# play-with-HOI-generation/HOIG

Hardware: AMD Instinct MI355X
Metric: HOGAN train images/sec at 256x256 (higher is better)
Workload: dtype f16x3 fwd (both operands split hi+lo on fp16, 3 MFMAs per product) / bf16x2 bwd (dy split hi+lo, weights and x single bf16, 2 MFMAs per product), f32 accumulate; 1 GPU; 256x256 HO3Dv3-shaped synthetic, batch 8 per GPU, G+D full step (generator_spade_attn, VGG19 surrogate weights); global_batch=8, parallelism=dp1

## Files before the change

hoig_amd/csrc/conv_thin.hip:

```cpp
#include "common.h"
#include <map>
#include <mutex>

namespace {

typedef _Float16 f16x8 __attribute__((ext_vector_type(8)));
typedef short s16x4 __attribute__((ext_vector_type(4)));

constexpr int TH = 4, TW = 32, NTHR = 256;

struct ThinArgs {
    const float *T;
    const float *D;
    const float *bias;
    float *Out;
    float *Ws;
    int Bn, H, W, F, CD, KS, pad;
    int flip;
    int sj, st, sf;
    int act;
    float slope;
    int accumulate;
    float wscale;
    int K, KP, N, NP;
    int tiles_x, tiles_y, ntiles, strip;
    int HR, CW;
    double *stats;
};

template <bool FP16>
__device__ __forceinline__ void split16(float x, unsigned short &hi, unsigned short &lo) {
    if (FP16) {
        const _Float16 h = (_Float16)x;
        const _Float16 l = (_Float16)(x - (float)h);
        hi = __builtin_bit_cast(unsigned short, h);
        lo = __builtin_bit_cast(unsigned short, l);
    } else {
        const __bf16 h = (__bf16)x;
        hi = __builtin_bit_cast(unsigned short, h);
        const __bf16 l = (__bf16)(x - hoig_bf2f(hi));
        lo = __builtin_bit_cast(unsigned short, l);
    }
}

template <bool FP16>
__device__ __forceinline__ f32x16 mfma16(const bf16x8 a, const bf16x8 b, const f32x16 c) {
    if (FP16) return __builtin_amdgcn_mfma_f32_32x32x16_f16(__builtin_bit_cast(f16x8, a), __builtin_bit_cast(f16x8, b), c, 0, 0, 0);
    return __builtin_amdgcn_mfma_f32_32x32x16_bf16(a, b, c, 0, 0, 0);
}

constexpr int HMAX = 12;
struct HaloRegs {
    float v[HMAX];
};
struct HaloMap {
    int lds[HMAX];
    int rc[HMAX];
    int rounds;
};
__device__ __forceinline__ void halo_map(const ThinArgs &p, HaloMap &m) {
    const int wr = TW + p.KS - 1;
    const int row_elems = wr * p.F;
    const int total = p.HR * row_elems;
    m.rounds = (total + NTHR - 1) / NTHR;
#pragma unroll
    for (int it = 0; it < HMAX; ++it) {
        const int i = threadIdx.x + it * NTHR;
        m.lds[it] = -1;
        m.rc[it] = 0;
        if (i < total) {
            const int hy = i / row_elems, e = i - hy * row_elems;
            const int hx = e / p.F, f = e - hx * p.F;
            m.lds[it] = (f * p.HR + hy) * p.CW + hx;
            m.rc[it] = hy | (hx << 8) | (f << 16);
        }
    }
}
__device__ __forceinline__ void halo_load(const ThinArgs &p, const HaloMap &m, int b, int y0, int x0, HaloRegs &h) {
    const float *img = p.T + (size_t)b * p.H * p.W * p.F;
#pragma unroll
    for (int it = 0; it < HMAX; ++it) {
        h.v[it] = 0.f;
        if (it < m.rounds && m.lds[it] >= 0) {
// ... 83 lines not shown
    const int t_end = min(p.ntiles, (int)(blockIdx.x + 1) * p.strip);
    HaloRegs hreg;
    HaloMap hmap;
    halo_map(p, hmap);
    {
        int b, y0, x0;
        tile_coords(p, blockIdx.x * p.strip, b, y0, x0);
        halo_load(p, hmap, b, y0, x0, hreg);
    }
    float st1[2] = {0.f, 0.f}, st2[2] = {0.f, 0.f};
    int sb = -1;
    auto flush_stats = [&]() {
        if (sb >= 0) {
#pragma unroll
            for (int j = 0; j < 2; ++j) {
                const float s1 = st1[j] + __shfl_xor(st1[j], 32), s2 = st2[j] + __shfl_xor(st2[j], 32);
                if (lh == 0) {
                    hoig_stats_add(p.stats, sb, p.CD, 0, cbase + j * 32 + l31, s1);
                    hoig_stats_add(p.stats, sb, p.CD, 1, cbase + j * 32 + l31, s2);
                }
                st1[j] = st2[j] = 0.f;
            }
        }
    };
    for (int t = blockIdx.x * p.strip; t < t_end; ++t) {
        int b, y0, x0;
        tile_coords(p, t, b, y0, x0);
        if (p.stats && b != sb) {
            flush_stats();
            sb = b;
        }
        __syncthreads();
        halo_store<FP16, NT>(p, hmap, hreg, Tl);
        __syncthreads();
        if (t + 1 < t_end) {
            int b2, y2, x2;
            tile_coords(p, t + 1, b2, y2, x2);
            halo_load(p, hmap, b2, y2, x2, hreg);
        }
        f32x16 acc[2];
#pragma unroll
        for (int j = 0; j < 2; ++j)
#pragma unroll
            for (int r = 0; r < 16; ++r) acc[j][r] = 0.f;
#pragma unroll 1
        for (int kk = 0; kk < ksteps; ++kk) {
            const int k0 = kk * 16 + lh * 8;
            const bf16x8 offs = *reinterpret_cast<const bf16x8 *>(toff + k0);
            bf16x8 a0, a1;
#pragma unroll
            for (int e = 0; e < 8; ++e) {
                const int o = (int)(unsigned short)offs[e] + pix;
                a0[e] = (short)Tl[o];
                if (NT == 2) a1[e] = (short)Tl[tplane + o];
            }
#pragma unroll
            for (int j = 0; j < 2; ++j) {
                const unsigned short *wr = Wl + (j * 32 + l31) * wstride + k0;
                const bf16x8 w0 = *reinterpret_cast<const bf16x8 *>(wr);
                if (NT == 2) acc[j] = mfma16<FP16>(a1, w0, acc[j]);
                if (NW == 2) acc[j] = mfma16<FP16>(a0, *reinterpret_cast<const bf16x8 *>(wr + 64 * wstride), acc[j]);
                acc[j] = mfma16<FP16>(a0, w0, acc[j]);
            }
        }
        const int oy = y0 + wave;
#pragma unroll
        for (int r = 0; r < 16; ++r) {
            const int ox = x0 + (r & 3) + 8 * (r >> 2) + 4 * lh;
            float *dst = p.Out + (((size_t)b * p.H + oy) * p.W + ox) * p.CD + cbase + l31;
#pragma unroll
            for (int j = 0; j < 2; ++j) {
                float v = acc[j][r] * inv + bias_r[j];
                v = fast_act(v, nslope, special, p.act, p.slope);
                if (p.accumulate) v += dst[j * 32];
                dst[j * 32] = v;
                st1[j] += v;
                st2[j] += v * v;
            }
        }
    }
    if (p.stats) flush_stats();
}

constexpr int DROW = 192;

template <int NPW, int WN, int NT, int ND>
__global__ __launch_bounds__(NTHR) void thin_wgrad_kernel(const ThinArgs p) {
    constexpr int WK = 4 / WN, NPIX = TH * TW, KSTEPS = NPIX / 16;
    extern __shared__ __attribute__((aligned(16))) unsigned char smem[];
    unsigned char *Dl = smem;
    unsigned short *Tl = reinterpret_cast<unsigned short *>(smem + ND * NPIX * DROW);
    float *Gl = reinterpret_cast<float *>(smem);
    const int tid = threadIdx.x, lane = tid & 63, wave = tid >> 6;
    const int l31 = lane & 31, lh = lane >> 5;
    const int wn = wave % WN, wk = wave / WN;
    const int cbase = blockIdx.y * 64;
    const int KK = p.KS * p.KS;
    const int tplane = p.F * p.HR * p.CW;

    int noff[NPW];
    bool nval[NPW];
#pragma unroll
    for (int j = 0; j < NPW; ++j) {
        const int n = (wn * NPW + j) * 32 + l31;
        nval[j] = n < p.N;
        const int nc = nval[j] ? n : 0;
        const int tap = nc / p.F, f = nc - tap * p.F;
        const int tt = p.flip ? KK - 1 - tap : tap;
        const int r = tt / p.KS, s = tt - r * p.KS;
        noff[j] = (f * p.HR + r) * p.CW + s + lh * 8;
    }
    const int g = lane >> 4, q = (lane >> 2) & 3, pp = lane & 3;
    const int a_off = (8 * (g >> 1) + q) * DROW + (16 * (g & 1) + 4 * pp) * 2;

    f32x16 acc[2][NPW];
#pragma unroll
    for (int i = 0; i < 2; ++i)
#pragma unroll
        for (int j = 0; j < NPW; ++j)
#pragma unroll
            for (int r = 0; r < 16; ++r) acc[i][j][r] = 0.f;

    constexpr int DT = NPIX * 8 / NTHR;
    float4 dreg[DT][2];
    auto load_d = [&](int t) {
        int b, y0, x0;
        tile_coords(p, t, b, y0, x0);
#pragma unroll
        for (int i = 0; i < DT; ++i) {
            const int task = tid + i * NTHR, px = task >> 3, c8 = task & 7;
            const int yy = y0 + (px >> 5), xx = x0 + (px & 31);
            const float *src = p.D + (((size_t)b * p.H + yy) * p.W + xx) * p.CD + cbase + c8 * 8;
            dreg[i][0] = *reinterpret_cast<const float4 *>(src);
            dreg[i][1] = *reinterpret_cast<const float4 *>(src + 4);
        }
    };
    auto store_d = [&]() {
#pragma unroll
        for (int i = 0; i < DT; ++i) {
            const int task = tid + i * NTHR, px = task >> 3, c8 = task & 7;
            const float v[8] = {dreg[i][0].x, dreg[i][0].y, dreg[i][0].z, dreg[i][0].w,
                                dreg[i][1].x, dreg[i][1].y, dreg[i][1].z, dreg[i][1].w};
            bf16x8 hi, lo;
#pragma unroll
            for (int e = 0; e < 8; e += 2) {
                typedef float f2v __attribute__((ext_vector_type(2)));
                typedef __bf16 b2v __attribute__((ext_vector_type(2)));
                const f2v x2 = {v[e], v[e + 1]};
                const unsigned hp = __builtin_bit_cast(unsigned, __builtin_convertvector(x2, b2v));
                hi[e] = (short)(hp & 0xffffu);
                hi[e + 1] = (short)(hp >> 16);
                if (ND == 2) {
                    const f2v r2 = {v[e] - __uint_as_float(hp << 16), v[e + 1] - __uint_as_float(hp & 0xffff0000u)};
                    const unsigned lp = __builtin_bit_cast(unsigned, __builtin_convertvector(r2, b2v));
                    lo[e] = (short)(lp & 0xffffu);
                    lo[e + 1] = (short)(lp >> 16);
                }
            }
            *reinterpret_cast<bf16x8 *>(Dl + px * DROW + c8 * 16) = hi;
            if (ND == 2) *reinterpret_cast<bf16x8 *>(Dl + NPIX * DROW + px * DROW + c8 * 16) = lo;
        }
    };

    int t = blockIdx.x;
    HaloRegs hreg;
    HaloMap hmap;
// ... 27 lines not shown
                    const s16x4 v0 = __builtin_amdgcn_ds_read_tr16_b64_v4i16((__attribute__((address_space(3))) s16x4 *)(src));
                    const s16x4 v1 = __builtin_amdgcn_ds_read_tr16_b64_v4i16((__attribute__((address_space(3))) s16x4 *)(src + 4 * DROW));
                    a[i][d] = (bf16x8){v0[0], v0[1], v0[2], v0[3], v1[0], v1[1], v1[2], v1[3]};
                }
            const int base = prow * p.CW + pcol;
#pragma unroll
            for (int j = 0; j < NPW; ++j) {
                bf16x8 b0, b1;
#pragma unroll
                for (int e = 0; e < 8; ++e) {
                    const int o = base + noff[j] + e;
                    b0[e] = nval[j] ? (short)Tl[o] : (short)0;
                    if (NT == 2) b1[e] = nval[j] ? (short)Tl[tplane + o] : (short)0;
                }
#pragma unroll
                for (int i = 0; i < 2; ++i) {
                    if (ND == 2) acc[i][j] = mfma16<false>(a[i][1], b0, acc[i][j]);
                    if (NT == 2) acc[i][j] = mfma16<false>(a[i][0], b1, acc[i][j]);
                    acc[i][j] = mfma16<false>(a[i][0], b0, acc[i][j]);
                }
            }
        }
    }

    __syncthreads();
    for (int i = tid; i < 64 * p.NP; i += NTHR) Gl[i] = 0.f;
    __syncthreads();
#pragma unroll
    for (int i = 0; i < 2; ++i)
#pragma unroll
        for (int j = 0; j < NPW; ++j) {
            const int n = (wn * NPW + j) * 32 + l31;
            if (n < p.NP)
#pragma unroll
                for (int r = 0; r < 16; ++r) {
                    const int m = i * 32 + (r & 3) + 8 * (r >> 2) + 4 * lh;
                    if (WK > 1) atomicAdd(&Gl[m * p.NP + n], acc[i][j][r]);
                    else Gl[m * p.NP + n] = acc[i][j][r];
                }
        }
    __syncthreads();
    if (p.Ws) {
        float *dst = p.Ws + ((size_t)blockIdx.y * gridDim.x + blockIdx.x) * 64 * p.NP;
        for (int i = tid; i < 64 * p.NP; i += NTHR) dst[i] = Gl[i];
        return;
    }
    if (p.sj == 1) {
        for (int i = tid; i < 64 * p.N; i += NTHR) {
            const int n = i >> 6, m = i & 63;
            const int tap = n / p.F, f = n - tap * p.F;
            atomicAdd(p.Out + (size_t)f * p.sf + (size_t)tap * p.st + cbase + m, Gl[m * p.NP + n]);
        }
    } else {
        for (int i = tid; i < 64 * p.N; i += NTHR) {
            const int m = i / p.N, n = i - m * p.N;
            const int tap = n / p.F, f = n - tap * p.F;
            atomicAdd(p.Out + (size_t)(cbase + m) * p.sj + (size_t)tap * p.st + (size_t)f * p.sf, Gl[m * p.NP + n]);
        }
    }
}

__global__ __launch_bounds__(NTHR) void thin_reduce_kernel(const ThinArgs p, int nwg) {
    const int cbase = blockIdx.y * 64;
    const float *src = p.Ws + (size_t)blockIdx.y * nwg * 64 * p.NP;
    const int i = blockIdx.x * NTHR + threadIdx.x;
    if (i >= 64 * p.N) return;
    const int m = i / p.N, n = i - m * p.N;
    const int wper = (nwg + (int)gridDim.z - 1) / (int)gridDim.z;
    const int w0 = blockIdx.z * wper, w1 = min(nwg, w0 + wper);
    const size_t step = (size_t)64 * p.NP;
    const float *col = src + m * p.NP + n + (size_t)w0 * step;
    float v0 = 0.f, v1 = 0.f, v2 = 0.f, v3 = 0.f;
    int w = w0;
    for (; w + 3 < w1; w += 4, col += 4 * step) {
        v0 += col[0];
        v1 += col[step];
        v2 += col[2 * step];
        v3 += col[3 * step];
    }
    for (; w < w1; ++w, col += step) v0 += col[0];
    const float v = (v0 + v1) + (v2 + v3);
    const int tap = n / p.F, f = n - tap * p.F;
    atomicAdd(p.Out + (size_t)(cbase + m) * p.sj + (size_t)tap * p.st + (size_t)f * p.sf, v);
}

constexpr size_t WS_SLOT_BYTES = (size_t)16 << 20;
float *thin_workspace(hipStream_t st, size_t bytes) { return static_cast<float *>(hoig_detail::stream_scratch(st, bytes)); }

typedef float f32x4v __attribute__((ext_vector_type(4)));

struct ThinOutArgs {
    const float *D, *Wt, *bias;
    float *Out;
    int Bn, H, W, F, CD, KS, pad, flip;
    int sf, st, sj;
    unsigned long long acts;
    float slope, wscale;
    int tiles_x, tiles_y, ntiles, strip, HR, HWc;
};

template <bool FP16>
__device__ __forceinline__ f32x4v mfma16x16(const bf16x8 a, const bf16x8 b, const f32x4v c) {
    if (FP16) return __builtin_amdgcn_mfma_f32_16x16x32_f16(__builtin_bit_cast(f16x8, a), __builtin_bit_cast(f16x8, b), c, 0, 0, 0);
    return __builtin_amdgcn_mfma_f32_16x16x32_bf16(a, b, c, 0, 0, 0);
}

template <bool FP16, int ND, int NW>
__global__ __launch_bounds__(NTHR) void thin_out_kernel(const ThinOutArgs p) {
    constexpr int PROW = 80, WROW = 144;
    extern __shared__ __attribute__((aligned(16))) unsigned char smem[];
    const int KK = p.KS * p.KS, hpix = p.HR * p.HWc;
    unsigned char *Wl = smem;
    unsigned char *Dl = smem + (size_t)NW * (p.CD >> 6) * p.F * KK * WROW;
    const int tid = threadIdx.x, lane = tid & 63, wave = tid >> 6;
    const int l15 = lane & 15, kg = lane >> 4;
    const int wplane = p.F * KK * WROW;

    for (int i0 = tid; i0 < p.F * KK * p.CD; i0 += 4 * NTHR) {
        float v[4];
        int dst[4];
#pragma unroll
        for (int u = 0; u < 4; ++u) {
            const int i = i0 + u * NTHR;
            v[u] = 0.f;
            dst[u] = -1;
            if (i < p.F * KK * p.CD) {
                const int j = i % p.CD, ft = i / p.CD;
                const int tap = ft % KK, f = ft / KK;
                const int tw = p.flip ? KK - 1 - tap : tap;
                v[u] = p.Wt[(size_t)f * p.sf + (size_t)tw * p.st + (size_t)j * p.sj];
                dst[u] = ((j >> 6) * p.F * KK + f * KK + tap) * WROW + (j & 63) * 2;
            }
        }
#pragma unroll
        for (int u = 0; u < 4; ++u)
            if (dst[u] >= 0) {
                unsigned short hi, lo;
                split16<FP16>(v[u] * p.wscale, hi, lo);
                *reinterpret_cast<unsigned short *>(Wl + dst[u]) = hi;
                if (NW == 2) *reinterpret_cast<unsigned short *>(Wl + (size_t)(p.CD >> 6) * wplane + dst[u]) = lo;
            }
    }

    int apix[2];
#pragma unroll
    for (int i = 0; i < 2; ++i) {
        const int g = 2 * wave + i;
        apix[i] = ((g >> 1) * p.HWc + 16 * (g & 1) + l15) * PROW + kg * 16;
    }
    const bool nvalid = l15 < p.F;
    const int wrow0 = l15 * KK * WROW + kg * 16;
    const float inv = 1.f / p.wscale;
    const int act_n = (int)((p.acts >> (4 * l15)) & 15);
    const float bias_n = (p.bias && nvalid) ? p.bias[l15] : 0.f;

    constexpr int HT = 12;
    float4 hreg[HT];
    auto halo_load = [&](int t, int kh) {
        int b, y0, x0;
        const int tx = t % p.tiles_x, r1 = t / p.tiles_x;
        b = r1 / p.tiles_y;
        y0 = (r1 % p.tiles_y) * TH;
        x0 = tx * TW;
#pragma unroll
        for (int it = 0; it < HT; ++it) {
            const int i = tid + it * NTHR;
// ... 39 lines not shown
            if (kh + 1 < nkh) halo_load(t, kh + 1);
            else if (t + 1 < t_end) halo_load(t + 1, 0);
            const unsigned char *wbase = Wl + (size_t)(kh >> 1) * wplane + wrow0 + (kh & 1) * 64;
#pragma unroll 1
            for (int tap = 0; tap < KK; ++tap) {
                const int r = tap / p.KS, s_ = tap - r * p.KS;
                const int toff = (r * p.HWc + s_) * PROW;
                bf16x8 bh = {0, 0, 0, 0, 0, 0, 0, 0}, bl = bh;
                if (nvalid) {
                    bh = *reinterpret_cast<const bf16x8 *>(wbase + tap * WROW);
                    if (NW == 2) bl = *reinterpret_cast<const bf16x8 *>(wbase + (size_t)(p.CD >> 6) * wplane + tap * WROW);
                }
#pragma unroll
                for (int i = 0; i < 2; ++i) {
                    const unsigned char *ap = Dl + apix[i] + toff;
                    const bf16x8 ah = *reinterpret_cast<const bf16x8 *>(ap);
                    if (ND == 2) acc[i] = mfma16x16<FP16>(*reinterpret_cast<const bf16x8 *>(ap + hpix * PROW), bh, acc[i]);
                    if (NW == 2) acc[i] = mfma16x16<FP16>(ah, bl, acc[i]);
                    acc[i] = mfma16x16<FP16>(ah, bh, acc[i]);
                }
            }
        }
        if (nvalid) {
            const int tx = t % p.tiles_x, r1 = t / p.tiles_x;
            const int b = r1 / p.tiles_y, y0 = (r1 % p.tiles_y) * TH, x0 = tx * TW;
#pragma unroll
            for (int i = 0; i < 2; ++i) {
                const int g = 2 * wave + i;
                const int oy = y0 + (g >> 1), oxb = x0 + 16 * (g & 1) + 4 * kg;
#pragma unroll
                for (int e = 0; e < 4; ++e) {
                    const float v = acc[i][e] * inv + bias_n;
                    p.Out[(((size_t)b * p.H + oy) * p.W + oxb + e) * p.F + l15] = hoig_act(v, act_n, p.slope);
                }
            }
        }
    }
}

bool thin_geometry(const hoig_conv_desc *d) {
    return !d->transposed && d->stride == 1 && d->R == d->S && (d->R & 1) && d->R <= 7 && 2 * d->pad == d->R - 1 &&
           d->Ho == d->Hi && d->Wo == d->Wi && (d->Hi % TH) == 0 && (d->Wi % TW) == 0;
}

void fill_common(ThinArgs &a, const hoig_conv_desc *d, int F, int CD) {
    a.Bn = d->B; a.H = d->Hi; a.W = d->Wi; a.F = F; a.CD = CD; a.KS = d->R; a.pad = d->pad;
    a.K = d->R * d->S * F;
    a.KP = (a.K + 15) / 16 * 16;
    a.N = a.K;
    a.NP = (a.N + 31) / 32 * 32;
    a.tiles_x = d->Wi / TW; a.tiles_y = d->Hi / TH;
    a.ntiles = d->B * a.tiles_x * a.tiles_y;
    a.HR = TH + d->R - 1;
    a.CW = (TW + d->R - 1 + 8 + 1) & ~1;
    a.bias = nullptr; a.act = HOIG_ACT_NONE; a.slope = 0.f; a.accumulate = 0; a.wscale = 1.f; a.strip = 1; a.Ws = nullptr; a.stats = nullptr;
}

template <bool FP16>
int launch_gemm(const ThinArgs &a, int precision, hipStream_t st) {
    const int nt = precision == HOIG_PREC_BF16 ? 1 : 2, nw = precision == HOIG_PREC_BF16X3 ? 2 : 1;
    const size_t smem = (size_t)nw * 64 * (a.KP + 8) * 2 + (size_t)a.KP * 2 + (size_t)nt * a.F * a.HR * a.CW * 2;
    if (smem > 160 * 1024) return HOIG_EUNSUPPORTED;
    dim3 grid((unsigned)hoig_cdiv(a.ntiles, a.strip), a.CD / 64);
    HOIG_ROUTE_FD(FP16, thin);
#define HOIG_THIN_GEMM(NT_, NW_)                                                                                         \
    do {                                                                                                                 \
        static hoig_once attr;                                                                                        \
        if (!attr.done()) {                                                                                                     \
            if (hipFuncSetAttribute(reinterpret_cast<const void *>(&thin_gemm_kernel<FP16, NT_, NW_>),                   \
                                    hipFuncAttributeMaxDynamicSharedMemorySize, 160 * 1024) != hipSuccess)               \
                return HOIG_ELAUNCH;                                                                                     \
            attr.set();                                                                                                 \
        }                                                                                                                \
        thin_gemm_kernel<FP16, NT_, NW_><<<grid, NTHR, smem, st>>>(a);                                                   \
    } while (0)
    if (nt == 2 && nw == 2) HOIG_THIN_GEMM(2, 2);
    else if (nt == 2) HOIG_THIN_GEMM(2, 1);
    else HOIG_THIN_GEMM(1, 1);
#undef HOIG_THIN_GEMM
    HOIG_LAUNCH_CHECK();
    return HOIG_OK;
}

template <int NPW, int WN>
int launch_wgrad_t(const ThinArgs &a, int nt, int nd, dim3 grid, size_t smem, hipStream_t st) {
#define HOIG_THIN_WG(NT_, ND_)                                                                                           \
    do {                                                                                                                 \
        static hoig_once attr;                                                                                        \
        if (!attr.done()) {                                                                                                     \
            if (hipFuncSetAttribute(reinterpret_cast<const void *>(&thin_wgrad_kernel<NPW, WN, NT_, ND_>),               \
                                    hipFuncAttributeMaxDynamicSharedMemorySize, 160 * 1024) != hipSuccess)               \
                return HOIG_ELAUNCH;                                                                                     \
            attr.set();                                                                                                 \
        }                                                                                                                \
        thin_wgrad_kernel<NPW, WN, NT_, ND_><<<grid, NTHR, smem, st>>>(a);                                               \
    } while (0)
    if (nt == 2 && nd == 2) HOIG_THIN_WG(2, 2);
    else if (nt == 2) HOIG_THIN_WG(2, 1);
    else if (nd == 2) HOIG_THIN_WG(1, 2);
    else HOIG_THIN_WG(1, 1);
#undef HOIG_THIN_WG
    HOIG_LAUNCH_CHECK();
    return HOIG_OK;
}

}

int hoig_conv_thin_fwd(const hoig_conv_desc *d, const float *x, const float *w, const float *bias, float *y, hipStream_t st, double *stats) {
    if (d->precision == HOIG_PREC_F32 || !thin_geometry(d) || d->Ci > (d->R <= 3 ? 12 : 8) || d->Ci < 1 || (d->Co % 64)) return HOIG_EUNSUPPORTED;
    ThinArgs a;
    fill_common(a, d, d->Ci, d->Co);
    a.T = x; a.D = w; a.bias = bias; a.Out = y; a.stats = stats;
    a.flip = 0;
    a.sj = d->R * d->S * d->Ci; a.st = d->Ci; a.sf = 1;
    a.act = d->act; a.slope = d->slope;
    a.wscale = 256.f;
    a.strip = a.ntiles >= 4096 ? 8 : (a.ntiles >= 1024 ? 4 : 1);
    return launch_gemm<true>(a, d->precision, st);
}

int hoig_conv_thin_dgrad(const hoig_conv_desc *d, const float *dy, const float *w, float *dx, int accumulate, hipStream_t st) {
    if (d->precision == HOIG_PREC_F32 || !thin_geometry(d) || d->Co > 8 || d->Co < 1 || (d->Ci % 64)) return HOIG_EUNSUPPORTED;
    ThinArgs a;
    fill_common(a, d, d->Co, d->Ci);
    a.T = dy; a.D = w; a.Out = dx;
    a.flip = 1;
    a.sj = 1; a.st = d->Ci; a.sf = d->R * d->S * d->Ci;
    a.accumulate = accumulate;
    a.strip = a.ntiles >= 4096 ? 8 : (a.ntiles >= 1024 ? 4 : 1);
    return launch_gemm<false>(a, d->precision, st);
}

bool hoig_conv_thin_wgrad_applies(const hoig_conv_desc *d) {
    if (d->precision == HOIG_PREC_F32 || !thin_geometry(d)) return false;
    return (d->Ci <= (d->R <= 3 ? 12 : 8) && (d->Co % 64) == 0) || (d->Co <= 8 && (d->Ci % 64) == 0);
}

int hoig_conv_thin_wgrad(const hoig_conv_desc *d, const float *x, const float *dy, float *dw, hipStream_t st) {
    if (d->precision == HOIG_PREC_F32 || !thin_geometry(d)) return HOIG_EUNSUPPORTED;
    const bool thin_in = d->Ci <= (d->R <= 3 ? 12 : 8) && (d->Co % 64) == 0, thin_out = d->Co <= 8 && (d->Ci % 64) == 0;
    if (!thin_in && !thin_out) return HOIG_EUNSUPPORTED;
    ThinArgs a;
    int nt, nd;
    if (thin_in) {
        fill_common(a, d, d->Ci, d->Co);
        a.T = x; a.D = dy; a.flip = 0;
        a.sj = d->R * d->S * d->Ci; a.st = d->Ci; a.sf = 1;
        nd = d->precision == HOIG_PREC_BF16 ? 1 : 2;
        nt = d->precision == HOIG_PREC_BF16X3 ? 2 : 1;
    } else {
        fill_common(a, d, d->Co, d->Ci);
        a.T = dy; a.D = x; a.flip = 1;
        a.sj = 1; a.st = d->Ci; a.sf = d->R * d->S * d->Ci;
        nt = d->precision == HOIG_PREC_BF16 ? 1 : 2;
        nd = d->precision == HOIG_PREC_BF16X3 ? 2 : 1;
    }
    a.Out = dw;
    const int nfr = a.NP / 32;
    if (nfr > 16) return HOIG_EUNSUPPORTED;
    size_t smem = (size_t)nd * TH * TW * DROW + (size_t)nt * a.F * a.HR * a.CW * 2;
    const size_t gsm = (size_t)64 * a.NP * 4;
    if (gsm > smem) smem = gsm;
    if (smem > 160 * 1024) return HOIG_EUNSUPPORTED;
    int nwg = 512;
    if (smem > 80 * 1024 || a.N >= 128) nwg = 256;
    if (nwg > a.ntiles) nwg = a.ntiles;
    const int groups = a.CD / 64;
    while (nwg > 64 && (size_t)nwg * groups * 64 * a.NP * 4 > WS_SLOT_BYTES) nwg >>= 1;
    dim3 grid(nwg, groups);
    a.Ws = nwg > 8 ? thin_workspace(st, (size_t)nwg * groups * 64 * a.NP * 4) : nullptr;
    if (thin_in) a.Ws ? HOIG_ROUTE_W(wgrad_thin_in_ws) : HOIG_ROUTE_W(wgrad_thin_in_direct);
    else a.Ws ? HOIG_ROUTE_W(wgrad_thin_out_ws) : HOIG_ROUTE_W(wgrad_thin_out_direct);
    int rc;
    if (nfr == 1) rc = launch_wgrad_t<1, 1>(a, nt, nd, grid, smem, st);
    else if (nfr == 2) rc = launch_wgrad_t<2, 1>(a, nt, nd, grid, smem, st);
    else if (nfr <= 4) rc = launch_wgrad_t<2, 2>(a, nt, nd, grid, smem, st);
    else if (nfr <= 8) rc = launch_wgrad_t<2, 4>(a, nt, nd, grid, smem, st);
    else rc = launch_wgrad_t<4, 4>(a, nt, nd, grid, smem, st);
    if (rc != HOIG_OK || !a.Ws) return rc;
    thin_reduce_kernel<<<dim3((unsigned)hoig_cdiv(64 * a.N, NTHR), groups, (unsigned)hoig_cdiv(nwg, 32)), NTHR, 0, st>>>(a, nwg);
    HOIG_LAUNCH_CHECK();
    return HOIG_OK;
}

int hoig_conv_thin_out(const hoig_conv_desc *d, const float *x, const float *w, const float *bias, float *y,
                       unsigned long long acts, int dgrad, hipStream_t st) {
    if (d->precision == HOIG_PREC_F32 || !thin_geometry(d)) return HOIG_EUNSUPPORTED;
    const int F = dgrad ? d->Ci : d->Co, CD = dgrad ? d->Co : d->Ci;
    if (F < 1 || F > 16 || (CD % 64)) return HOIG_EUNSUPPORTED;
    if (d->R > 3) return HOIG_EUNSUPPORTED;
    ThinOutArgs a;
    a.D = x; a.Wt = w; a.bias = bias; a.Out = y;
    a.Bn = d->B; a.H = d->Hi; a.W = d->Wi; a.F = F; a.CD = CD; a.KS = d->R; a.pad = d->pad;
    const int KK = d->R * d->S;
    if (!dgrad) { a.flip = 0; a.sf = KK * CD; a.st = CD; a.sj = 1; a.wscale = 256.f; }
    else { a.flip = 1; a.sf = 1; a.st = F; a.sj = KK * F; a.wscale = 1.f; }
    a.acts = acts; a.slope = d->slope;
    a.tiles_x = d->Wi / TW; a.tiles_y = d->Hi / TH; a.ntiles = d->B * a.tiles_x * a.tiles_y;
    a.strip = a.ntiles >= 2048 ? 8 : (a.ntiles >= 512 ? 2 : 1);
    a.HR = TH + d->R - 1; a.HWc = TW + d->R - 1;
    if (a.HR * a.HWc * 8 > 12 * NTHR) return HOIG_EUNSUPPORTED;
    const int nd = d->precision == HOIG_PREC_BF16 ? 1 : 2, nw = d->precision == HOIG_PREC_BF16X3 ? 2 : 1;
    const size_t smem = (size_t)nw * (CD / 64) * F * KK * 144 + (size_t)nd * a.HR * a.HWc * 80;
    if (smem > 160 * 1024) return HOIG_EUNSUPPORTED;
    const unsigned grid = (unsigned)hoig_cdiv(a.ntiles, a.strip);
    HOIG_ROUTE_FD(!dgrad, thin_out);
#define HOIG_THIN_OUT(FP16_, ND_, NW_)                                                                                   \
    do {                                                                                                                 \
        static hoig_once attr;                                                                                        \
        if (!attr.done()) {                                                                                                     \
            if (hipFuncSetAttribute(reinterpret_cast<const void *>(&thin_out_kernel<FP16_, ND_, NW_>),                   \
                                    hipFuncAttributeMaxDynamicSharedMemorySize, 160 * 1024) != hipSuccess)               \
                return HOIG_ELAUNCH;                                                                                     \
            attr.set();                                                                                                 \
        }                                                                                                                \
        thin_out_kernel<FP16_, ND_, NW_><<<grid, NTHR, smem, st>>>(a);                                                   \
    } while (0)
    if (!dgrad) {
        if (nd == 2 && nw == 2) HOIG_THIN_OUT(true, 2, 2);
        else if (nd == 2) HOIG_THIN_OUT(true, 2, 1);
        else HOIG_THIN_OUT(true, 1, 1);
    } else {
        if (nd == 2 && nw == 2) HOIG_THIN_OUT(false, 2, 2);
        else if (nd == 2) HOIG_THIN_OUT(false, 2, 1);
        else HOIG_THIN_OUT(false, 1, 1);
    }
#undef HOIG_THIN_OUT
    HOIG_LAUNCH_CHECK();
    return HOIG_OK;
}
```

hoig_amd/csrc/tuning.h:

```cpp
#pragma once
enum HoigTuning { HOIG_TUNE_IGEMM16 = 0, HOIG_TUNE_S2_16, HOIG_TUNE_FLAT5, HOIG_TUNE_WFLAT5, HOIG_TUNE_HEAD16, HOIG_TUNE_D_EARLY, HOIG_TUNE_SPLIT_GRADS, HOIG_TUNE_PAIR, HOIG_TUNE_WDMA16, HOIG_TUNE_S2_PIPE, HOIG_TUNE_NORM_IN, HOIG_TUNE_WINO8, HOIG_TUNE_HALO5, HOIG_TUNE_COUNT };
int hoig_tuning(int id);
```

hoig_amd/csrc/tuning.hip:

```cpp
#include <cstring>
#include "hoig_kernels.h"
#include "tuning.h"
#include "conv_route.h"

namespace {
struct Entry {
    const char *key;
    int value;
};
Entry g_table[HOIG_TUNE_COUNT] = {
    {"igemm16", 1},
    {"s2_16", 1},
    {"flat5", 2},
    {"wflat5", 1},
    {"head16", 1},
    {"d_early", 1},
    {"split_grads", 1},
    {"pair", 2},
    {"wdma16", 2},
    {"s2_pipe", 1},
    {"norm_in", 1},
    {"wino8", 0},
    {"halo5", 1},
};
}

int hoig_tuning(int id) { return (id >= 0 && id < HOIG_TUNE_COUNT) ? g_table[id].value : 0; }

extern "C" int hoig_set_tuning(const char *key, int value) {
    if (!key) return -1;
    for (int i = 0; i < HOIG_TUNE_COUNT; ++i)
        if (strcmp(g_table[i].key, key) == 0) {
            const int prev = g_table[i].value;
            if (value >= 0) g_table[i].value = value;
            return prev;
        }
    return -1;
}

thread_local int hoig_route_last[3] = {0, 0, 0};

extern "C" int hoig_conv_last_route(int which) { return (which >= 0 && which < 3) ? hoig_route_last[which] : -1; }

extern "C" const char *hoig_conv_route_name(int id) {
    static const char *const names[HOIG_ROUTE_COUNT] = {
        "none",
#define HOIG_R_W(n) #n,
#define HOIG_R_D(n) "dgrad_" #n,
#define HOIG_R_F(n) "fwd_" #n,
#define HOIG_R_FD(n) "fwd_" #n, "dgrad_" #n,
        HOIG_CONV_ROUTES(HOIG_R_W, HOIG_R_D, HOIG_R_F, HOIG_R_FD)
#undef HOIG_R_W
#undef HOIG_R_D
#undef HOIG_R_F
#undef HOIG_R_FD
    };
    return (id >= 0 && id < HOIG_ROUTE_COUNT) ? names[id] : nullptr;
}
```

Measured before the change: 131.1 images/s.

## Add thin16 padded-channel layout kernels for thin conv fwd, dgrad and wgrad

Adds a new family of thin-channel convolution kernels that pad the small channel count to 4/8/16 and pack the halo into a row-contiguous LDS layout. Forward and dgrad use 16x16x32 MFMAs with 512 threads, 8-row tiles and register-prefetched halos, while wgrad uses transposed LDS reads over the new layout. The goal is fewer wasted K-steps and cheaper fragment loads for low-channel convs. The cost is extra padding work, more LDS, and a selection table (thin16_selected) that gates which shapes take the new path.

```diff
diff --git a/hoig_amd/csrc/conv_thin.hip b/hoig_amd/csrc/conv_thin.hip
--- a/hoig_amd/csrc/conv_thin.hip
+++ b/hoig_amd/csrc/conv_thin.hip
@@ -1,4 +1,6 @@
 #include "common.h"
+#include "conv_thin16_tables.h"
+#include "tuning.h"
 #include <map>
 #include <mutex>
 
@@ -248,6 +250,244 @@
     if (p.stats) flush_stats();
 }
 
+constexpr int TH16 = 8, NTHR16 = 512;
+
+typedef unsigned int u32x2 __attribute__((ext_vector_type(2)));
+
+template <bool A16>
+__device__ __forceinline__ bf16x8 lds_frag(const unsigned short *src) {
+    if (A16) return *reinterpret_cast<const bf16x8 *>(src);
+    const u32x2 v0 = *reinterpret_cast<const u32x2 *>(src), v1 = *reinterpret_cast<const u32x2 *>(src + 4);
+    typedef unsigned int u32x4 __attribute__((ext_vector_type(4)));
+    return __builtin_bit_cast(bf16x8, (u32x4){v0[0], v0[1], v1[0], v1[1]});
+}
+
+template <bool FP16>
+__device__ __forceinline__ f32x4 mfma16x32(const bf16x8 a, const bf16x8 b, const f32x4 c) {
+    if (FP16) return __builtin_amdgcn_mfma_f32_16x16x32_f16(__builtin_bit_cast(f16x8, a), __builtin_bit_cast(f16x8, b), c, 0, 0, 0);
+    return __builtin_amdgcn_mfma_f32_16x16x32_bf16(a, b, c, 0, 0, 0);
+}
+
+constexpr int HMAX16 = 9;
+template <int HM>
+struct Halo16 {
+    float v[HM];
+    int rc[HM];
+};
+template <int NTH, int HM>
+__device__ __forceinline__ void halo16_map(const ThinArgs &p, const Thin16Geom &g, Halo16<HM> &m) {
+    const int wr = TW + p.KS - 1;
+    const int row_elems = wr * p.F;
+    const int total = g.HR * row_elems;
+#pragma unroll
+    for (int it = 0; it < HM; ++it) {
+        const int i = threadIdx.x + it * NTH;
+        m.rc[it] = -1;
+        if (i < total) {
+            const int hy = i / row_elems, e = i - hy * row_elems;
+            const int hx = e / p.F, f = e - hx * p.F;
+            m.rc[it] = hy | (hx << 8) | (f << 16);
+        }
+    }
+}
+template <int HM>
+__device__ __forceinline__ void halo16_load(const ThinArgs &p, Halo16<HM> &m, int b, int y0, int x0) {
+    const float *img = p.T + (size_t)b * p.H * p.W * p.F;
+#pragma unroll
+    for (int it = 0; it < HM; ++it) {
+        m.v[it] = 0.f;
+        if (m.rc[it] >= 0) {
+            const int gy = y0 - p.pad + (m.rc[it] & 255), gx = x0 - p.pad + ((m.rc[it] >> 8) & 255);
+            if (gy >= 0 && gy < p.H && gx >= 0 && gx < p.W) m.v[it] = img[((size_t)gy * p.W + gx) * p.F + (m.rc[it] >> 16)];
+        }
+    }
+}
+template <bool FP16, int NT, int HM>
+__device__ __forceinline__ void halo16_store(const Thin16Geom &g, const Halo16<HM> &m, unsigned short *Tl, int plane) {
+#pragma unroll
+    for (int it = 0; it < HM; ++it)
+        if (m.rc[it] >= 0) {
+            unsigned short hi, lo;
+            split16<FP16>(m.v[it], hi, lo);
+            const int o = thin16_halo_elem(g, m.rc[it] & 255, (m.rc[it] >> 8) & 255, m.rc[it] >> 16);
+            Tl[o] = hi;
+            if (NT == 2) Tl[plane + o] = lo;
+        }
+}
+
+template <bool FP16, int NT, int NW, bool A16, bool STATS>
+__global__ __launch_bounds__(NTHR16) void thin16_gemm_kernel(const ThinArgs p, const Thin16Geom g) {
+    extern __shared__ __attribute__((aligned(16))) unsigned char smem[];
+    const int wstride = g.KP + 8;
+    unsigned short *Wl = reinterpret_cast<unsigned short *>(smem);
+    unsigned short *Tl = Wl + NW * 64 * wstride;
+    const int tid = threadIdx.x, lane = tid & 63, wave = tid >> 6;
+    const int l15 = lane & 15, lg = lane >> 4;
+    const int cbase = blockIdx.y * 64;
+    const int tplane = g.HR * g.CWE;
+
+    for (int i0 = tid; i0 < 64 * g.KP; i0 += 4 * NTHR16) {
+        float v[4];
+        int dst[4];
+#pragma unroll
+        for (int u = 0; u < 4; ++u) {
+            const int i = i0 + u * NTHR16;
+            v[u] = 0.f;
+            dst[u] = -1;
+            if (i < 64 * g.KP) {
+                const int n = i / g.KP, k = i - n * g.KP;
+                dst[u] = n * wstride + k;
+                const long long src = thin16_weight_index(g, k, cbase + n, p.sj, p.st, p.sf, p.flip);
+                if (src >= 0) v[u] = p.D[src];
+            }
+        }
+#pragma unroll
+        for (int u = 0; u < 4; ++u)
+            if (dst[u] >= 0) {
+                unsigned short hi, lo;
+                split16<FP16>(v[u] * p.wscale, hi, lo);
+                Wl[dst[u]] = hi;
+                if (NW == 2) Wl[64 * wstride + dst[u]] = lo;
+            }
+    }
+    for (int i = tid; i < NT * tplane; i += NTHR16) Tl[i] = 0;
+
+    const float nslope = p.act == HOIG_ACT_NONE ? 1.f : (p.act == HOIG_ACT_RELU ? 0.f : p.slope);
+    const bool special = p.act == HOIG_ACT_TANH || p.act == HOIG_ACT_SIGMOID;
+    const float inv = 1.f / p.wscale;
+    const int ksteps = g.KP >> 5, spr = g.KRP >> 5;
+    const unsigned short *wlane = Wl + l15 * wstride + lg * 8;
+    const unsigned short *tlane = Tl + wave * g.CWE + l15 * g.FP + lg * 8;
+
+    const int t_end = min(p.ntiles, (int)(blockIdx.x + 1) * p.strip);
+    Halo16<HMAX16> halo;
+    halo16_map<NTHR16>(p, g, halo);
+    auto coords = [&](int t, int &b, int &y0, int &x0) {
+        const int tx = t % p.tiles_x;
+        t /= p.tiles_x;
+        b = t / p.tiles_y;
+        y0 = (t - b * p.tiles_y) * TH16;
+        x0 = tx * TW;
+    };
+    {
+        int b, y0, x0;
+        coords(blockIdx.x * p.strip, b, y0, x0);
+        halo16_load(p, halo, b, y0, x0);
+    }
+    float st1[4][4], st2[4][4];
+#pragma unroll
+    for (int mt = 0; mt < 4; ++mt)
+#pragma unroll
+        for (int e = 0; e < 4; ++e) st1[mt][e] = st2[mt][e] = 0.f;
+    int sb = -1;
+    auto flush_stats = [&]() {
+        if (STATS && sb >= 0) {
+#pragma unroll
+            for (int mt = 0; mt < 4; ++mt)
+#pragma unroll
+                for (int e = 0; e < 4; ++e) {
+                    float s1 = st1[mt][e], s2 = st2[mt][e];
+#pragma unroll
+                    for (int o = 1; o < 16; o <<= 1) {
+                        s1 += __shfl_xor(s1, o);
+                        s2 += __shfl_xor(s2, o);
+                    }
+                    if (l15 == 0) {
+                        hoig_stats_add(p.stats, sb, p.CD, 0, cbase + mt * 16 + lg * 4 + e, s1);
+                        hoig_stats_add(p.stats, sb, p.CD, 1, cbase + mt * 16 + lg * 4 + e, s2);
+                    }
+                    st1[mt][e] = st2[mt][e] = 0.f;
+                }
+        }
+    };
+    struct Frags {
+        bf16x8 w[4][NW], t[2][NT];
+    };
+    for (int t = blockIdx.x * p.strip; t < t_end; ++t) {
+        int b, y0, x0;
+        coords(t, b, y0, x0);
+        if (STATS && b != sb) {
+            flush_stats();
+            sb = b;
+        }
+        __syncthreads();
+        halo16_store<FP16, NT>(g, halo, Tl, tplane);
+        __syncthreads();
+        if (t + 1 < t_end) {
+            int b2, y2, x2;
+            coords(t + 1, b2, y2, x2);
+            halo16_load(p, halo, b2, y2, x2);
+        }
+        const int oy = y0 + wave;
+        if (oy >= p.H) continue;
+        f32x4 acc[4][2];
+#pragma unroll
+        for (int mt = 0; mt < 4; ++mt)
+#pragma unroll
+            for (int nt = 0; nt < 2; ++nt) acc[mt][nt] = (f32x4){0.f, 0.f, 0.f, 0.f};
+        auto load = [&](Frags &f, int kk) {
+            const int r = spr == 1 ? kk : kk >> 1;
+            const unsigned short *tp = tlane + r * g.CWE + (kk - r * spr) * 32;
+            const unsigned short *wp = wlane + kk * 32;
+#pragma unroll
+            for (int nt = 0; nt < 2; ++nt) {
+                f.t[nt][0] = lds_frag<A16>(tp + nt * 16 * g.FP);
+                if (NT == 2) f.t[nt][NT - 1] = lds_frag<A16>(tp + tplane + nt * 16 * g.FP);
+            }
+#pragma unroll
+            for (int mt = 0; mt < 4; ++mt) {
+                f.w[mt][0] = *reinterpret_cast<const bf16x8 *>(wp + mt * 16 * wstride);
+                if (NW == 2) f.w[mt][NW - 1] = *reinterpret_cast<const bf16x8 *>(wp + (64 + mt * 16) * wstride);
+            }
+        };
+        auto mma = [&](const Frags &f) {
+#pragma unroll
+            for (int mt = 0; mt < 4; ++mt)
+#pragma unroll
+                for (int nt = 0; nt < 2; ++nt) {
+                    if (NT == 2) acc[mt][nt] = mfma16x32<FP16>(f.w[mt][0], f.t[nt][NT - 1], acc[mt][nt]);
+                    if (NW == 2) acc[mt][nt] = mfma16x32<FP16>(f.w[mt][NW - 1], f.t[nt][0], acc[mt][nt]);
+                    acc[mt][nt] = mfma16x32<FP16>(f.w[mt][0], f.t[nt][0], acc[mt][nt]);
+                }
+        };
+        Frags f0, f1;
+        load(f0, 0);
+#pragma unroll 1
+        for (int kk = 0; kk < ksteps; kk += 2) {
+            if (kk + 1 < ksteps) load(f1, kk + 1);
+            mma(f0);
+            if (kk + 1 < ksteps) {
+                if (kk + 2 < ksteps) load(f0, kk + 2);
+                mma(f1);
+            }
+        }
+#pragma unroll
+        for (int nt = 0; nt < 2; ++nt) {
+            float *dst = p.Out + (((size_t)b * p.H + oy) * p.W + x0 + nt * 16 + l15) * p.CD + cbase + lg * 4;
+#pragma unroll
+            for (int mt = 0; mt < 4; ++mt) {
+                float4 o = make_float4(0.f, 0.f, 0.f, 0.f), bi = o;
+                if (p.accumulate) o = *reinterpret_cast<const float4 *>(dst + mt * 16);
+                if (p.bias) bi = *reinterpret_cast<const float4 *>(p.bias + cbase + mt * 16 + lg * 4);
+                float v[4] = {o.x, o.y, o.z, o.w};
+                const float bv[4] = {bi.x, bi.y, bi.z, bi.w};
+#pragma unroll
+                for (int e = 0; e < 4; ++e) {
+                    float u = acc[mt][nt][e] * inv + bv[e];
+                    u = fast_act(u, nslope, special, p.act, p.slope);
+                    v[e] += u;
+                    if (STATS) {
+                        st1[mt][e] += v[e];
+                        st2[mt][e] += v[e] * v[e];
+                    }
+                }
+                *reinterpret_cast<float4 *>(dst + mt * 16) = make_float4(v[0], v[1], v[2], v[3]);
+            }
+        }
+    }
+    if (STATS) flush_stats();
+}
+
 constexpr int DROW = 192;
 
 template <int NPW, int WN, int NT, int ND>
@@ -441,6 +681,188 @@
     const float v = (v0 + v1) + (v2 + v3);
     const int tap = n / p.F, f = n - tap * p.F;
     atomicAdd(p.Out + (size_t)(cbase + m) * p.sj + (size_t)tap * p.st + (size_t)f * p.sf, v);
+}
+
+template <int NPW, int WN, int NT, int ND>
+__global__ __launch_bounds__(NTHR) void thin16_wgrad_kernel(const ThinArgs p, const Thin16Geom g) {
+    constexpr int WK = 4 / WN, NPIX = TH * TW, KSTEPS = NPIX / 16;
+    extern __shared__ __attribute__((aligned(16))) unsigned char smem[];
+    unsigned char *Dl = smem;
+    unsigned short *Tl = reinterpret_cast<unsigned short *>(smem + ND * NPIX * DROW);
+    float *Gl = reinterpret_cast<float *>(smem);
+    const int tid = threadIdx.x, lane = tid & 63, wave = tid >> 6;
+    const int l31 = lane & 31, lh = lane >> 5;
+    const int wn = wave % WN, wk = wave / WN;
+    const int cbase = blockIdx.y * 64;
+    const int KK = p.KS * p.KS;
+    const int tplane = g.HR * g.CWE;
+    const int fpr = g.KRP >> 5, nfr = p.KS * fpr, NC = nfr * 32;
+
+    int coff[NPW];
+    bool cval[NPW];
+#pragma unroll
+    for (int j = 0; j < NPW; ++j) {
+        const int c = j * WN + wn;
+        cval[j] = c < nfr;
+        const int r = cval[j] ? c / fpr : 0, q = cval[j] ? c - r * fpr : 0;
+        coff[j] = (r * g.CWE + q * 32) * 2;
+    }
+    const int gq = lane >> 4, q4 = (lane >> 2) & 3, pp = lane & 3;
+    const int a_off = (8 * (gq >> 1) + q4) * DROW + (16 * (gq & 1) + 4 * pp) * 2;
+    const int prow_b = g.FP * 2;
+    const int b_off = (8 * (gq >> 1) + q4) * prow_b + (16 * (gq & 1) + 4 * pp) * 2;
+
+    f32x16 acc[2][NPW];
+#pragma unroll
+    for (int i = 0; i < 2; ++i)
+#pragma unroll
+        for (int j = 0; j < NPW; ++j)
+#pragma unroll
+            for (int r = 0; r < 16; ++r) acc[i][j][r] = 0.f;
+
+    constexpr int DT = NPIX * 8 / NTHR;
+    float4 dreg[DT][2];
+    auto load_d = [&](int t) {
+        int b, y0, x0;
+        tile_coords(p, t, b, y0, x0);
+#pragma unroll
+        for (int i = 0; i < DT; ++i) {
+            const int task = tid + i * NTHR, px = task >> 3, c8 = task & 7;
+            const int yy = y0 + (px >> 5), xx = x0 + (px & 31);
+            const float *src = p.D + (((size_t)b * p.H + yy) * p.W + xx) * p.CD + cbase + c8 * 8;
+            dreg[i][0] = *reinterpret_cast<const float4 *>(src);
+            dreg[i][1] = *reinterpret_cast<const float4 *>(src + 4);
+        }
+    };
+    auto store_d = [&]() {
+#pragma unroll
+        for (int i = 0; i < DT; ++i) {
+            const int task = tid + i * NTHR, px = task >> 3, c8 = task & 7;
+            const float v[8] = {dreg[i][0].x, dreg[i][0].y, dreg[i][0].z, dreg[i][0].w,
+                                dreg[i][1].x, dreg[i][1].y, dreg[i][1].z, dreg[i][1].w};
+            bf16x8 hi, lo;
+#pragma unroll
+            for (int e = 0; e < 8; e += 2) {
+                typedef float f2v __attribute__((ext_vector_type(2)));
+                typedef __bf16 b2v __attribute__((ext_vector_type(2)));
+                const f2v x2 = {v[e], v[e + 1]};
+                const unsigned hp = __builtin_bit_cast(unsigned, __builtin_convertvector(x2, b2v));
+                hi[e] = (short)(hp & 0xffffu);
+                hi[e + 1] = (short)(hp >> 16);
+                if (ND == 2) {
+                    const f2v r2 = {v[e] - __uint_as_float(hp << 16), v[e + 1] - __uint_as_float(hp & 0xffff0000u)};
+                    const unsigned lp = __builtin_bit_cast(unsigned, __builtin_convertvector(r2, b2v));
+                    lo[e] = (short)(lp & 0xffffu);
+                    lo[e + 1] = (short)(lp >> 16);
+                }
+            }
+            *reinterpret_cast<bf16x8 *>(Dl + px * DROW + c8 * 16) = hi;
+            if (ND == 2) *reinterpret_cast<bf16x8 *>(Dl + NPIX * DROW + px * DROW + c8 * 16) = lo;
+        }
+    };
+    auto read_tr = [&](const unsigned char *src, int step) {
+        const s16x4 v0 = __builtin_amdgcn_ds_read_tr16_b64_v4i16((__attribute__((address_space(3))) s16x4 *)(src));
+        const s16x4 v1 = __builtin_amdgcn_ds_read_tr16_b64_v4i16((__attribute__((address_space(3))) s16x4 *)(src + step));
+        return (bf16x8){v0[0], v0[1], v0[2], v0[3], v1[0], v1[1], v1[2], v1[3]};
+    };
+
+    for (int i = tid; i < NT * tplane; i += NTHR) Tl[i] = 0;
+
+    int t = blockIdx.x;
+    Halo16<HMAX> halo;
+    halo16_map<NTHR>(p, g, halo);
+    if (t < p.ntiles) {
+        int b, y0, x0;
+        tile_coords(p, t, b, y0, x0);
+        load_d(t);
+        halo16_load(p, halo, b, y0, x0);
+    }
+    for (; t < p.ntiles; t += gridDim.x) {
+        __syncthreads();
+        store_d();
+        halo16_store<false, NT>(g, halo, Tl, tplane);
+        __syncthreads();
+        if (t + (int)gridDim.x < p.ntiles) {
+            int b, y0, x0;
+            tile_coords(p, t + gridDim.x, b, y0, x0);
+            load_d(t + gridDim.x);
+            halo16_load(p, halo, b, y0, x0);
+        }
+#pragma unroll 1
+        for (int ks = wk; ks < KSTEPS; ks += WK) {
+            const int prow = ks >> 1, pcol = (ks & 1) * 16;
+            bf16x8 a[2][ND];
+#pragma unroll
+            for (int i = 0; i < 2; ++i)
+#pragma unroll
+                for (int d = 0; d < ND; ++d)
+                    a[i][d] = read_tr(Dl + d * NPIX * DROW + (prow * 32 + pcol) * DROW + a_off + i * 64, 4 * DROW);
+            const unsigned char *tb = reinterpret_cast<const unsigned char *>(Tl) + (prow * g.CWE + pcol * g.FP) * 2 + b_off;
+#pragma unroll
+            for (int j = 0; j < NPW; ++j) {
+                if (!cval[j]) continue;
+                const bf16x8 b0 = read_tr(tb + coff[j], 4 * prow_b);
+                bf16x8 b1 = b0;
+                if (NT == 2) b1 = read_tr(tb + tplane * 2 + coff[j], 4 * prow_b);
+#pragma unroll
+                for (int i = 0; i < 2; ++i) {
+                    if (ND == 2) acc[i][j] = mfma16<false>(a[i][ND - 1], b0, acc[i][j]);
+                    if (NT == 2) acc[i][j] = mfma16<false>(a[i][0], b1, acc[i][j]);
+                    acc[i][j] = mfma16<false>(a[i][0], b0, acc[i][j]);
+                }
+            }
+        }
+    }
+
+    __syncthreads();
+    for (int i = tid; i < 64 * NC; i += NTHR) Gl[i] = 0.f;
+    __syncthreads();
+#pragma unroll
+    for (int i = 0; i < 2; ++i)
+#pragma unroll
+        for (int j = 0; j < NPW; ++j) {
+            if (!cval[j]) continue;
+            const int n = (j * WN + wn) * 32 + l31;
+#pragma unroll
+            for (int r = 0; r < 16; ++r) {
+                const int m = i * 32 + (r & 3) + 8 * (r >> 2) + 4 * lh;
+                if (WK > 1) atomicAdd(&Gl[m * NC + n], acc[i][j][r]);
+                else Gl[m * NC + n] = acc[i][j][r];
+            }
+        }
+    __syncthreads();
+    auto col_of = [&](int n, int &tap, int &f) {
+        tap = n / p.F;
+        f = n - tap * p.F;
+        const int tt = p.flip ? KK - 1 - tap : tap;
+        const int r = tt / p.KS, s_ = tt - r * p.KS;
+        return r * g.KRP + s_ * g.FP + f;
+    };
+    if (p.Ws) {
+        float *dst = p.Ws + ((size_t)blockIdx.y * gridDim.x + blockIdx.x) * 64 * p.NP;
+        for (int i = tid; i < 64 * p.N; i += NTHR) {
+            const int m = i / p.N, n = i - m * p.N;
+            int tap, f;
+            const int c = col_of(n, tap, f);
+            dst[m * p.NP + n] = Gl[m * NC + c];
+        }
+        return;
+    }
+    if (p.sj == 1) {
+        for (int i = tid; i < 64 * p.N; i += NTHR) {
+            const int n = i >> 6, m = i & 63;
+            int tap, f;
+            const int c = col_of(n, tap, f);
+            atomicAdd(p.Out + (size_t)f * p.sf + (size_t)tap * p.st + cbase + m, Gl[m * NC + c]);
+        }
+    } else {
+        for (int i = tid; i < 64 * p.N; i += NTHR) {
+            const int m = i / p.N, n = i - m * p.N;
+            int tap, f;
+            const int c = col_of(n, tap, f);
+            atomicAdd(p.Out + (size_t)(cbase + m) * p.sj + (size_t)tap * p.st + (size_t)f * p.sf, Gl[m * NC + c]);
+        }
+    }
 }
 
 constexpr size_t WS_SLOT_BYTES = (size_t)16 << 20;
@@ -646,6 +1068,68 @@
     return HOIG_OK;
 }
 
+enum { T16_FWD = 0, T16_DGRAD, T16_WGRAD_IN, T16_WGRAD_OUT };
+bool thin16_selected(int pass, int KS, int FP) {
+    const int v = hoig_tuning(HOIG_TUNE_THIN16);
+    if (v != 1) return v >= 2;
+    switch (pass) {
+        case T16_FWD:
+        case T16_DGRAD: return KS == 7 && FP <= 8;
+        case T16_WGRAD_IN: return (KS == 7 && FP <= 8) || (KS == 3 && FP == 16);
+        case T16_WGRAD_OUT: return KS == 7 && FP == 4;
+    }
+    return false;
+}
+
+int thin_strip(int automatic) {
+    const int v = hoig_tuning(HOIG_TUNE_THIN_STRIP);
+    return v > 0 ? v : automatic;
+}
+
+template <bool FP16>
+int launch_gemm16(ThinArgs a, int precision, hipStream_t st) {
+    const int nt = precision == HOIG_PREC_BF16 ? 1 : 2, nw = precision == HOIG_PREC_BF16X3 ? 2 : 1;
+    const Thin16Geom g = thin16_geom(a.KS, a.F, TH16, TW);
+    if (g.KRP > 64 || g.HR * (TW + a.KS - 1) * a.F > HMAX16 * NTHR16) return HOIG_EUNSUPPORTED;
+    a.tiles_y = (a.H + TH16 - 1) / TH16;
+    a.ntiles = a.Bn * a.tiles_x * a.tiles_y;
+    const int per_cu = (int)hoig_cdiv(a.ntiles, 256);
+    a.strip = thin_strip(per_cu < 1 ? 1 : (per_cu > 16 ? 16 : per_cu));
+    const size_t smem = (size_t)nw * 64 * (g.KP + 8) * 2 + (size_t)nt * g.HR * g.CWE * 2;
+    if (smem > 160 * 1024) return HOIG_EUNSUPPORTED;
+    dim3 grid((unsigned)hoig_cdiv(a.ntiles, a.strip), a.CD / 64);
+    HOIG_ROUTE_FD(FP16, thin);
+#define HOIG_THIN16_GEMM_S(NT_, NW_, A16_, ST_)                                                                               \
+    do {                                                                                                                 \
+        static hoig_once attr;                                                                                        \
+        if (!attr.done()) {                                                                                                     \
+            if (hipFuncSetAttribute(reinterpret_cast<const void *>(&thin16_gemm_kernel<FP16, NT_, NW_, A16_, ST_>),      \
+                                    hipFuncAttributeMaxDynamicSharedMemorySize, 160 * 1024) != hipSuccess)               \
+                return HOIG_ELAUNCH;                                                                                     \
+            attr.set();                                                                                                 \
+        }                                                                                                                \
+        thin16_gemm_kernel<FP16, NT_, NW_, A16_, ST_><<<grid, NTHR16, smem, st>>>(a, g);                                 \
+    } while (0)
+#define HOIG_THIN16_GEMM(NT_, NW_, A16_)                                                                                 \
+    do {                                                                                                                 \
+        if (FP16 && a.stats) HOIG_THIN16_GEMM_S(NT_, NW_, A16_, FP16);                                                   \
+        else HOIG_THIN16_GEMM_S(NT_, NW_, A16_, false);                                                                  \
+    } while (0)
+    if (g.FP >= 8) {
+        if (nt == 2 && nw == 2) HOIG_THIN16_GEMM(2, 2, true);
+        else if (nt == 2) HOIG_THIN16_GEMM(2, 1, true);
+        else HOIG_THIN16_GEMM(1, 1, true);
+    } else {
+        if (nt == 2 && nw == 2) HOIG_THIN16_GEMM(2, 2, false);
+        else if (nt == 2) HOIG_THIN16_GEMM(2, 1, false);
+        else HOIG_THIN16_GEMM(1, 1, false);
+    }
+#undef HOIG_THIN16_GEMM
+#undef HOIG_THIN16_GEMM_S
+    HOIG_LAUNCH_CHECK();
+    return HOIG_OK;
+}
+
 template <int NPW, int WN>
 int launch_wgrad_t(const ThinArgs &a, int nt, int nd, dim3 grid, size_t smem, hipStream_t st) {
 #define HOIG_THIN_WG(NT_, ND_)                                                                                           \
@@ -668,6 +1152,28 @@
     return HOIG_OK;
 }
 
+template <int NPW, int WN>
+int launch_wgrad16_t(const ThinArgs &a, const Thin16Geom &g, int nt, int nd, dim3 grid, size_t smem, hipStream_t st) {
+#define HOIG_THIN_WG(NT_, ND_)                                                                                           \
+    do {                                                                                                                 \
+        static hoig_once attr;                                                                                        \
+        if (!attr.done()) {                                                                                                     \
+            if (hipFuncSetAttribute(reinterpret_cast<const void *>(&thin16_wgrad_kernel<NPW, WN, NT_, ND_>),             \
+                                    hipFuncAttributeMaxDynamicSharedMemorySize, 160 * 1024) != hipSuccess)               \
+                return HOIG_ELAUNCH;                                                                                     \
+            attr.set();                                                                                                 \
+        }                                                                                                                \
+        thin16_wgrad_kernel<NPW, WN, NT_, ND_><<<grid, NTHR, smem, st>>>(a, g);                                          \
+    } while (0)
+    if (nt == 2 && nd == 2) HOIG_THIN_WG(2, 2);
+    else if (nt == 2) HOIG_THIN_WG(2, 1);
+    else if (nd == 2) HOIG_THIN_WG(1, 2);
+    else HOIG_THIN_WG(1, 1);
+#undef HOIG_THIN_WG
+    HOIG_LAUNCH_CHECK();
+    return HOIG_OK;
+}
+
 }
 
 int hoig_conv_thin_fwd(const hoig_conv_desc *d, const float *x, const float *w, const float *bias, float *y, hipStream_t st, double *stats) {
@@ -679,7 +1185,11 @@
     a.sj = d->R * d->S * d->Ci; a.st = d->Ci; a.sf = 1;
     a.act = d->act; a.slope = d->slope;
     a.wscale = 256.f;
-    a.strip = a.ntiles >= 4096 ? 8 : (a.ntiles >= 1024 ? 4 : 1);
+    if (thin16_selected(T16_FWD, a.KS, thin16_fp(a.F))) {
+        const int rc = launch_gemm16<true>(a, d->precision, st);
+        if (rc != HOIG_EUNSUPPORTED) return rc;
+    }
+    a.strip = thin_strip(a.ntiles >= 4096 ? 8 : (a.ntiles >= 1024 ? 4 : 1));
     return launch_gemm<true>(a, d->precision, st);
 }
 
@@ -691,7 +1201,11 @@
     a.flip = 1;
     a.sj = 1; a.st = d->Ci; a.sf = d->R * d->S * d->Ci;
     a.accumulate = accumulate;
-    a.strip = a.ntiles >= 4096 ? 8 : (a.ntiles >= 1024 ? 4 : 1);
+    if (thin16_selected(T16_DGRAD, a.KS, thin16_fp(a.F))) {
+        const int rc = launch_gemm16<false>(a, d->precision, st);
+        if (rc != HOIG_EUNSUPPORTED) return rc;
+    }
+    a.strip = thin_strip(a.ntiles >= 4096 ? 8 : (a.ntiles >= 1024 ? 4 : 1));
     return launch_gemm<false>(a, d->precision, st);
 }
 
@@ -720,10 +1234,13 @@
         nd = d->precision == HOIG_PREC_BF16X3 ? 2 : 1;
     }
     a.Out = dw;
-    const int nfr = a.NP / 32;
+    const Thin16Geom g = thin16_geom(a.KS, a.F, TH, TW);
+    const int nfr16 = a.KS * (g.KRP / 32);
+    const bool t16 = thin16_selected(thin_in ? T16_WGRAD_IN : T16_WGRAD_OUT, a.KS, g.FP) && nfr16 <= 16 && g.HR * (TW + a.KS - 1) * a.F <= HMAX * NTHR;
+    const int nfr = t16 ? nfr16 : a.NP / 32;
     if (nfr > 16) return HOIG_EUNSUPPORTED;
-    size_t smem = (size_t)nd * TH * TW * DROW + (size_t)nt * a.F * a.HR * a.CW * 2;
-    const size_t gsm = (size_t)64 * a.NP * 4;
+    size_t smem = (size_t)nd * TH * TW * DROW + (size_t)nt * (t16 ? g.HR * g.CWE : a.F * a.HR * a.CW) * 2;
+    const size_t gsm = (size_t)64 * (t16 ? nfr16 * 32 : a.NP) * 4;
     if (gsm > smem) smem = gsm;
     if (smem > 160 * 1024) return HOIG_EUNSUPPORTED;
     int nwg = 512;
@@ -736,7 +1253,13 @@
     if (thin_in) a.Ws ? HOIG_ROUTE_W(wgrad_thin_in_ws) : HOIG_ROUTE_W(wgrad_thin_in_direct);
     else a.Ws ? HOIG_ROUTE_W(wgrad_thin_out_ws) : HOIG_ROUTE_W(wgrad_thin_out_direct);
     int rc;
-    if (nfr == 1) rc = launch_wgrad_t<1, 1>(a, nt, nd, grid, smem, st);
+    if (t16) {
+        if (nfr == 1) rc = launch_wgrad16_t<1, 1>(a, g, nt, nd, grid, smem, st);
+        else if (nfr == 2) rc = launch_wgrad16_t<2, 1>(a, g, nt, nd, grid, smem, st);
+        else if (nfr <= 4) rc = launch_wgrad16_t<2, 2>(a, g, nt, nd, grid, smem, st);
+        else if (nfr <= 8) rc = launch_wgrad16_t<2, 4>(a, g, nt, nd, grid, smem, st);
+        else rc = launch_wgrad16_t<4, 4>(a, g, nt, nd, grid, smem, st);
+    } else if (nfr == 1) rc = launch_wgrad_t<1, 1>(a, nt, nd, grid, smem, st);
     else if (nfr == 2) rc = launch_wgrad_t<2, 1>(a, nt, nd, grid, smem, st);
     else if (nfr <= 4) rc = launch_wgrad_t<2, 2>(a, nt, nd, grid, smem, st);
     else if (nfr <= 8) rc = launch_wgrad_t<2, 4>(a, nt, nd, grid, smem, st);
diff --git a/hoig_amd/csrc/conv_thin16_tables.h b/hoig_amd/csrc/conv_thin16_tables.h
--- /dev/null
+++ b/hoig_amd/csrc/conv_thin16_tables.h
@@ -0,0 +1,50 @@
+#pragma once
+
+#if defined(__HIPCC__)
+#define HOIG_T16_HD __host__ __device__ __forceinline__
+#else
+#define HOIG_T16_HD inline
+#endif
+
+struct Thin16Geom {
+    int KS, F, FP;
+    int KRP;
+    int KP;
+    int HR;
+    int CWE;
+};
+
+HOIG_T16_HD int thin16_fp(int F) { return F <= 4 ? 4 : (F <= 8 ? 8 : 16); }
+
+HOIG_T16_HD Thin16Geom thin16_geom(int KS, int F, int th, int tw) {
+    Thin16Geom g;
+    g.KS = KS; g.F = F; g.FP = thin16_fp(F);
+    g.KRP = (KS * g.FP + 31) / 32 * 32;
+    g.KP = KS * g.KRP;
+    g.HR = th + KS - 1;
+    g.CWE = ((tw - 1) * g.FP + g.KRP + 7) / 8 * 8;
+    return g;
+}
+
+HOIG_T16_HD bool thin16_decode(const Thin16Geom &g, int k, int &r, int &s, int &f) {
+    r = k / g.KRP;
+    const int kr = k - r * g.KRP;
+    s = kr / g.FP;
+    f = kr - s * g.FP;
+    return s < g.KS && f < g.F;
+}
+
+HOIG_T16_HD long long thin16_weight_index(const Thin16Geom &g, int k, int j, long long sj, long long st, long long sf, int flip) {
+    int r, s, f;
+    if (!thin16_decode(g, k, r, s, f)) return -1;
+    const int tap = r * g.KS + s;
+    const int tw = flip ? g.KS * g.KS - 1 - tap : tap;
+    return j * sj + tw * st + f * sf;
+}
+
+HOIG_T16_HD int thin16_halo_offset(const Thin16Geom &g, int y, int x, int k) {
+    const int r = k / g.KRP;
+    return (y + r) * g.CWE + x * g.FP + (k - r * g.KRP);
+}
+
+HOIG_T16_HD int thin16_halo_elem(const Thin16Geom &g, int hy, int hx, int f) { return hy * g.CWE + hx * g.FP + f; }
diff --git a/hoig_amd/csrc/tuning.h b/hoig_amd/csrc/tuning.h
--- a/hoig_amd/csrc/tuning.h
+++ b/hoig_amd/csrc/tuning.h
@@ -1,3 +1,3 @@
 #pragma once
-enum HoigTuning { HOIG_TUNE_IGEMM16 = 0, HOIG_TUNE_S2_16, HOIG_TUNE_FLAT5, HOIG_TUNE_WFLAT5, HOIG_TUNE_HEAD16, HOIG_TUNE_D_EARLY, HOIG_TUNE_SPLIT_GRADS, HOIG_TUNE_PAIR, HOIG_TUNE_WDMA16, HOIG_TUNE_S2_PIPE, HOIG_TUNE_NORM_IN, HOIG_TUNE_WINO8, HOIG_TUNE_HALO5, HOIG_TUNE_COUNT };
+enum HoigTuning { HOIG_TUNE_IGEMM16 = 0, HOIG_TUNE_S2_16, HOIG_TUNE_FLAT5, HOIG_TUNE_WFLAT5, HOIG_TUNE_HEAD16, HOIG_TUNE_D_EARLY, HOIG_TUNE_SPLIT_GRADS, HOIG_TUNE_PAIR, HOIG_TUNE_WDMA16, HOIG_TUNE_S2_PIPE, HOIG_TUNE_NORM_IN, HOIG_TUNE_WINO8, HOIG_TUNE_HALO5, HOIG_TUNE_THIN16, HOIG_TUNE_THIN_STRIP, HOIG_TUNE_COUNT };
 int hoig_tuning(int id);
diff --git a/hoig_amd/csrc/tuning.hip b/hoig_amd/csrc/tuning.hip
--- a/hoig_amd/csrc/tuning.hip
+++ b/hoig_amd/csrc/tuning.hip
@@ -22,6 +22,8 @@
     {"norm_in", 1},
     {"wino8", 0},
     {"halo5", 1},
+    {"thin16", 1},
+    {"thin_strip", 0},
 };
 }
 
```

Result: no change. 131.6 images/s, median of 6 (+0.4%).
